# jianzhangcs/DAGL

Hardware: AMD Instinct MI355X
Metric: graph-attn fwd query-patches/s @256x256x64 k=8 (higher is better)
Workload: dtype f32

## Files before the change

### dagl_amd/csrc/prologue.hip

```cpp
#include <stdlib.h>

#include "dagl_common.h"
#include "thr_bias4.h"

namespace dagl {

constexpr int PC = 64;
constexpr int PRO_TW = 64;
constexpr int PRO_LW = PRO_TW + 2;
constexpr int PRO_LS = 68;
constexpr int PRO_ROWS = 4;

__global__ __launch_bounds__(256) void conv_pair_kernel(int H, int W, int rows_per_block,
                                                        const float* __restrict__ x,
                                                        const float* __restrict__ g_w, const float* __restrict__ g_b,
                                                        const float* __restrict__ th_w, const float* __restrict__ th_b,
                                                        float* __restrict__ b1p, float* __restrict__ b2p,
                                                        unsigned short* __restrict__ b1hi,
                                                        unsigned short* __restrict__ b1lo) {
    __shared__ __attribute__((aligned(16))) float ring[PRO_ROWS][PC][PRO_LS];
    const int tid = threadIdx.x;
    const int wave = __builtin_amdgcn_readfirstlane(tid >> 6);
    const int lane = tid & 63;
    const int i = lane & 15, g = lane >> 4;
    const int b = blockIdx.z;
    const int x0 = blockIdx.x * PRO_TW;
    const int y0 = blockIdx.y * rows_per_block;
    int y1 = y0 + rows_per_block; if (y1 > H) y1 = H;
    const int Hp = H + 2 * PADPIX, Wp = W + 2 * PADPIX;
    const float* xb = x + (size_t)b * PC * H * W;

    float wg[9][16], wt[16];
    {
        float* wl = &ring[0][0][0];
        for (int e = tid; e < 16 * PC * 9 / 4; e += 256)
            reinterpret_cast<float4*>(wl)[e] = reinterpret_cast<const float4*>(g_w)[e];
        for (int e = tid; e < 16 * PC / 4; e += 256)
            reinterpret_cast<float4*>(wl + 16 * PC * 9)[e] = reinterpret_cast<const float4*>(th_w)[e];
        __syncthreads();
#pragma unroll
        for (int tap = 0; tap < 9; ++tap)
#pragma unroll
            for (int T = 0; T < 16; ++T) wg[tap][T] = wl[(i * PC + 4 * T + g) * 9 + tap];
#pragma unroll
        for (int T = 0; T < 16; ++T) wt[T] = wl[16 * PC * 9 + i * PC + 4 * T + g];
        __syncthreads();
    }
    const float bias1 = g_b[i], bias2 = th_b[i];

    constexpr int NST = (PC * PRO_LW + 255) / 256;
    float st[NST];
    auto stage_load = [&](int yy) {
#pragma unroll
        for (int j = 0; j < NST; ++j) {
            const int idx = tid + 256 * j;
            const int ch = idx / PRO_LW, p = idx - ch * PRO_LW;
            const int xx = x0 - 1 + p;
            const bool ok = (idx < PC * PRO_LW) && (yy >= 0) && (yy < H) && (xx >= 0) && (xx < W);
            const int yc = yy < 0 ? 0 : (yy >= H ? H - 1 : yy), xc = xx < 0 ? 0 : (xx >= W ? W - 1 : xx);
            const int cc = ch < PC ? ch : PC - 1;
            const float raw = xb[((size_t)cc * H + yc) * W + xc];
            st[j] = ok ? raw : 0.f;
        }
    };
    auto stage_store = [&](int yy) {
        const int slot = (yy + 1) & (PRO_ROWS - 1);
#pragma unroll
        for (int j = 0; j < NST; ++j) {
            const int idx = tid + 256 * j;
            const int ch = idx / PRO_LW, p = idx - ch * PRO_LW;
            if (idx < PC * PRO_LW) ring[slot][ch][p] = st[j];
        }
    };

    stage_load(y0 - 1); stage_store(y0 - 1);
    stage_load(y0);     stage_store(y0);
    stage_load(y0 + 1); stage_store(y0 + 1);
    __syncthreads();

    const int px0 = 16 * wave;
    for (int y = y0; y < y1; ++y) {
        if (y + 1 < y1) stage_load(y + 2);
        f32x4 a0 = {0.f, 0.f, 0.f, 0.f}, a1 = a0, a2 = a0, at = a0;
#pragma unroll
        for (int T = 0; T < 16; ++T) {
            const int ch = 4 * T + g;
            const float* r0 = &ring[(y + 0) & 3][ch][px0 + i];
            const float* r1 = &ring[(y + 1) & 3][ch][px0 + i];
            const float* r2 = &ring[(y + 2) & 3][ch][px0 + i];
            const float c1 = r1[1];
            a0 = __builtin_amdgcn_mfma_f32_16x16x4f32(r0[0], wg[0][T], a0, 0, 0, 0);
            a1 = __builtin_amdgcn_mfma_f32_16x16x4f32(r1[0], wg[3][T], a1, 0, 0, 0);
            a2 = __builtin_amdgcn_mfma_f32_16x16x4f32(r2[0], wg[6][T], a2, 0, 0, 0);
            at = __builtin_amdgcn_mfma_f32_16x16x4f32(c1, wt[T], at, 0, 0, 0);
            a0 = __builtin_amdgcn_mfma_f32_16x16x4f32(r0[1], wg[1][T], a0, 0, 0, 0);
            a1 = __builtin_amdgcn_mfma_f32_16x16x4f32(c1, wg[4][T], a1, 0, 0, 0);
            a2 = __builtin_amdgcn_mfma_f32_16x16x4f32(r2[1], wg[7][T], a2, 0, 0, 0);
            a0 = __builtin_amdgcn_mfma_f32_16x16x4f32(r0[2], wg[2][T], a0, 0, 0, 0);
            a1 = __builtin_amdgcn_mfma_f32_16x16x4f32(r1[2], wg[5][T], a1, 0, 0, 0);
            a2 = __builtin_amdgcn_mfma_f32_16x16x4f32(r2[2], wg[8][T], a2, 0, 0, 0);
        }
#pragma unroll
        for (int r = 0; r < 4; ++r) {
            const int xx = x0 + px0 + 4 * g + r;
            if (xx < W) {
                const size_t o = (((size_t)b * Hp + y + PADPIX) * Wp + xx + PADPIX) * CH + i;
                const float v1 = ((a0[r] + a1[r]) + a2[r]) + bias1;
                if (b1p != nullptr) b1p[o] = v1;
                if (b1hi != nullptr) {
                    const float vs = v1 * 16.0f;
                    const _Float16 hh = (_Float16)vs;
                    const _Float16 ll = (_Float16)(vs - (float)hh);
                    b1hi[o] = __builtin_bit_cast(unsigned short, hh);
                    b1lo[o] = __builtin_bit_cast(unsigned short, ll);
                }
                b2p[o] = at[r] + bias2;
            }
        }
        if (y + 1 < y1) stage_store(y + 2);
        __syncthreads();
    }
}

typedef _Float16 h16x8 __attribute__((ext_vector_type(8)));
typedef _Float16 h16x4 __attribute__((ext_vector_type(4)));
constexpr int C16_PXB = 272;
constexpr int C16_ROWB = PRO_LW * C16_PXB;
constexpr int C16_WOFF = PRO_ROWS * C16_ROWB;
constexpr int C16_WB = (18 + 2) * 16 * 128;
constexpr float C16_XS = 16.0f, C16_WS = 256.0f;

__device__ __forceinline__ void c16_split(float v, _Float16& hi, _Float16& lo) {
    hi = (_Float16)v;
    lo = (_Float16)(v - (float)hi);
}

__global__ __launch_bounds__(256) void pack_conv_weight16_kernel(const float* __restrict__ g_w, const float* __restrict__ th_w,
                                                                 unsigned char* __restrict__ img) {
    const int e = blockIdx.x * 256 + threadIdx.x;
    if (e >= 16 * PC * 9 + 16 * PC) return;
    float v; int o, c, kb;
    if (e < 16 * PC * 9) {
        o = e / (PC * 9); const int rem = e - o * (PC * 9);
        c = rem / 9; const int tap = rem - c * 9;
        v = g_w[e]; kb = tap * 2 + (c >> 5);
    } else {
        const int t = e - 16 * PC * 9;
        o = t / PC; c = t - o * PC;
        v = th_w[t]; kb = 18 + (c >> 5);
    }
    _Float16 h, l;
    c16_split(v * C16_WS, h, l);
    unsigned char* d = img + (kb * 16 + o) * 128 + (c & 7) * 2;
    const int ks = (c & 31) >> 3, gs = (o >> 1) & 7;
    *reinterpret_cast<_Float16*>(d + ((ks ^ gs) << 4)) = h;
    *reinterpret_cast<_Float16*>(d + (((4 + ks) ^ gs) << 4)) = l;
    if (!(fabsf(v) * C16_WS < RANGE_LIMIT)) *reinterpret_cast<int32_t*>(img + C16_WB) = 1;
}

int launch_pack_conv_weight16(hipStream_t s, const float* g_w, const float* th_w, unsigned char* img) {
    DAGL_HIP_TRY(hipMemsetAsync(img + C16_WB, 0, 16, s));
    hipLaunchKernelGGL(pack_conv_weight16_kernel, dim3((16 * PC * 9 + 16 * PC + 255) / 256), dim3(256), 0, s, g_w, th_w, img);
    DAGL_LAUNCH_CHECK("pack_conv_weight16_kernel");
    return DAGL_OK;
}

__global__ __launch_bounds__(256) void conv_pair16_kernel(int H, int W, int rows_per_block, ConvHeadSet hs,
                                                          float* __restrict__ b2p, float* __restrict__ b1p, unsigned short* __restrict__ b1hi,
                                                          unsigned short* __restrict__ b1lo, uint32_t* __restrict__ clear_a,
                                                          int clear_a_words, uint32_t* __restrict__ clear_b, int clear_b_words,
                                                          RangeTag range, unsigned long long* times) {
    __shared__ __attribute__((aligned(16))) unsigned char smem[C16_WOFF + C16_WB + 16];
    int* const oor = reinterpret_cast<int*>(smem + C16_WOFF + C16_WB);
    const int tid = threadIdx.x;
    const int blin = (blockIdx.z * gridDim.y + blockIdx.y) * gridDim.x + blockIdx.x;
    dbg_stamp(times, blin, 0);
    float amax = 0.f;
    if (blockIdx.x == 0 && blockIdx.y == 0 && blockIdx.z == 0) {
        for (int t = tid; t < clear_a_words; t += 256) clear_a[t] = 0u;
        for (int t = tid; t < clear_b_words; t += 256) clear_b[t] = 0u;
    }
    if (tid == 0) *oor = 0;
    const int wave = __builtin_amdgcn_readfirstlane(tid >> 6);
    const int lane = tid & 63;
    const int i = lane & 15, kg = lane >> 4;
    const int b = blockIdx.z;
    const int head = b / hs.imgs;
    const float* __restrict__ x = hs.x[head];
    const unsigned char* __restrict__ wimg = hs.w[head];
    const float* __restrict__ g_b = hs.gb[head];
    const float* __restrict__ th_b = hs.tb[head];
    const int x0 = blockIdx.x * PRO_TW;
    const int y0 = blockIdx.y * rows_per_block;
    int y1 = y0 + rows_per_block; if (y1 > H) y1 = H;
    const int Hp = H + 2 * PADPIX, Wp = W + 2 * PADPIX;
    const float* xb = x + (size_t)(b - head * hs.imgs) * PC * H * W;

    const int hpx = 64 + (tid >> 6), hch = tid & 63;
    auto load_row = [&](int yy, float* st, float& sh) {
        const bool rok = (yy >= 0) && (yy < H);
        const int xa = x0 - 1 + lane, xc = x0 - 1 + hpx;
        const bool oka = rok && xa >= 0 && xa < W;
        const bool okc = rok && xc < W;
        const int yc = yy < 0 ? 0 : (yy >= H ? H - 1 : yy);
        const int xac = xa < 0 ? 0 : (xa >= W ? W - 1 : xa);
        const float* rp = xb + ((size_t)(16 * wave) * H + yc) * W + xac;
        float raw[16];
#pragma unroll
        for (int c = 0; c < 16; ++c) raw[c] = rp[(size_t)c * H * W];
        const float rh = xb[((size_t)hch * H + yc) * W + (xc >= W ? W - 1 : xc)];
#pragma unroll
        for (int c = 0; c < 16; ++c) st[c] = oka ? raw[c] : 0.f;
        sh = okc ? rh : 0.f;
    };
    float xs = C16_XS;
    float amax_x = 0.f;
    auto store_row = [&](int yy, const float* st, float sh) {
        unsigned char* row = smem + ((yy + 1) & (PRO_ROWS - 1)) * C16_ROWB;
        unsigned char* px = row + lane * C16_PXB;
        h16x8 hi0, hi1, lo0, lo1;
#pragma unroll
        for (int c = 0; c < 8; ++c) {
            _Float16 h, l;
            c16_split(st[c] * xs, h, l); hi0[c] = h; lo0[c] = l;
            c16_split(st[c + 8] * xs, h, l); hi1[c] = h; lo1[c] = l;
            amax_x = fmaxf(amax_x, fmaxf(fabsf(st[c]), fabsf(st[c + 8])));
        }
        *reinterpret_cast<h16x8*>(px + 32 * wave) = hi0;
        *reinterpret_cast<h16x8*>(px + 32 * wave + 16) = hi1;
        *reinterpret_cast<h16x8*>(px + 128 + 32 * wave) = lo0;
        *reinterpret_cast<h16x8*>(px + 128 + 32 * wave + 16) = lo1;
        if (tid < 128) {
            _Float16 h, l;
            c16_split(sh * xs, h, l);
            amax_x = fmaxf(amax_x, fabsf(sh));
            *reinterpret_cast<_Float16*>(row + hpx * C16_PXB + 2 * hch) = h;
            *reinterpret_cast<_Float16*>(row + hpx * C16_PXB + 128 + 2 * hch) = l;
        }
    };

    float st0[16], st1[16], st2[16], sh0, sh1, sh2;
    unsigned b1_bits = 0u;
    const bool tiers = hs.tiers.amax != nullptr;
    unsigned short* __restrict__ b1hi2 = hs.tiers.hi2;
    unsigned short* __restrict__ b1lo2 = hs.tiers.lo2;
    bool first = true;
    auto run_strip = [&]() {
    load_row(y0 - 1, st0, sh0);
    load_row(y0, st1, sh1);
    load_row(y0 + 1, st2, sh2);
    if (first) {
        uint4 wv[10];
#pragma unroll
        for (int j = 0; j < 10; ++j) wv[j] = reinterpret_cast<const uint4*>(wimg)[tid + 256 * j];
        if (tid == 0 && *reinterpret_cast<const int32_t*>(wimg + C16_WB) != 0) amax = __builtin_inff();
#pragma unroll
        for (int j = 0; j < 10; ++j) reinterpret_cast<uint4*>(smem + C16_WOFF)[tid + 256 * j] = wv[j];
    }
    store_row(y0 - 1, st0, sh0);
    store_row(y0, st1, sh1);
    store_row(y0 + 1, st2, sh2);
    __syncthreads();

    float bg[4], bt[4];
#pragma unroll
    for (int r = 0; r < 4; ++r) { bg[r] = g_b[4 * kg + r]; bt[r] = th_b[4 * kg + r]; }
    const unsigned char* wbase = smem + C16_WOFF + i * 128;
    const int whi = (kg ^ ((i >> 1) & 7)) << 4, wlo = ((4 + kg) ^ ((i >> 1) & 7)) << 4;
    const int pxo = (16 * wave + i) * C16_PXB + kg * 16;
    const float inv = 1.0f / (xs * C16_WS);
    h16x8 wh[20], wl2[20];
#pragma unroll
    for (int kb = 0; kb < 20; ++kb) {
        wh[kb] = *reinterpret_cast<const h16x8*>(wbase + kb * 2048 + whi);
        wl2[kb] = *reinterpret_cast<const h16x8*>(wbase + kb * 2048 + wlo);
    }
    b1_bits = 0u;

    dbg_stamp(times, blin, 1);
    if (y0 + 2 < y1 + 1) load_row(y0 + 2, st0, sh0);
    auto do_row = [&](int y, float* stc, float& shc, float* stn, float& shn) {
        if (y + 2 < y1) load_row(y + 3, stn, shn);
        f32x4 am[3][2], ac[3][2], tm[2], tc[2];
        const f32x4 zero4 = {0.f, 0.f, 0.f, 0.f};
#pragma unroll
        for (int u = 0; u < 3; ++u) { am[u][0] = zero4; am[u][1] = zero4; ac[u][0] = zero4; ac[u][1] = zero4; }
        tm[0] = zero4; tm[1] = zero4; tc[0] = zero4; tc[1] = zero4;
#pragma unroll
        for (int dx = 0; dx < 3; ++dx) {
#pragma unroll
            for (int dy = 0; dy < 3; ++dy) {
                const unsigned char* rowp = smem + ((y + dy) & (PRO_ROWS - 1)) * C16_ROWB + pxo;
#pragma unroll
                for (int cb = 0; cb < 2; ++cb) {
                    const int kb = (dy * 3 + dx) * 2 + cb;
                    const h16x8 w_hi = wh[kb], w_lo = wl2[kb];
                    const h16x8 p_hi = *reinterpret_cast<const h16x8*>(rowp + dx * C16_PXB + cb * 64);
                    const h16x8 p_lo = *reinterpret_cast<const h16x8*>(rowp + dx * C16_PXB + 128 + cb * 64);
                    ac[dy][cb] = __builtin_amdgcn_mfma_f32_16x16x32_f16(w_hi, p_lo, ac[dy][cb], 0, 0, 0);
                    am[dy][cb] = __builtin_amdgcn_mfma_f32_16x16x32_f16(w_hi, p_hi, am[dy][cb], 0, 0, 0);
                    ac[dy][cb] = __builtin_amdgcn_mfma_f32_16x16x32_f16(w_lo, p_hi, ac[dy][cb], 0, 0, 0);
                    if (dy == 1 && dx == 1) {
                        const h16x8 t_hi = wh[18 + cb], t_lo = wl2[18 + cb];
                        tc[cb] = __builtin_amdgcn_mfma_f32_16x16x32_f16(t_hi, p_lo, tc[cb], 0, 0, 0);
                        tm[cb] = __builtin_amdgcn_mfma_f32_16x16x32_f16(t_hi, p_hi, tm[cb], 0, 0, 0);
                        tc[cb] = __builtin_amdgcn_mfma_f32_16x16x32_f16(t_lo, p_hi, tc[cb], 0, 0, 0);
                    }
                }
            }
        }
        f32x4 ag, at;
#pragma unroll
        for (int r = 0; r < 4; ++r) {
            const float cr = ((ac[0][0][r] + ac[0][1][r]) + (ac[1][0][r] + ac[1][1][r])) + (ac[2][0][r] + ac[2][1][r]);
            const float mn = ((am[0][0][r] + am[0][1][r]) + (am[1][0][r] + am[1][1][r])) + (am[2][0][r] + am[2][1][r]);
            ag[r] = mn + cr;
            at[r] = (tm[0][r] + tm[1][r]) + (tc[0][r] + tc[1][r]);
        }
        const int xx = x0 + 16 * wave + i;
        if (xx < W) {
            const size_t o = (((size_t)b * Hp + y + PADPIX) * Wp + xx + PADPIX) * CH + 4 * kg;
            h16x4 vh, vl, vh2, vl2;
            float4 v2, v1q;
            float* v2p = &v2.x;
            float* v1p = &v1q.x;
#pragma unroll
            for (int r = 0; r < 4; ++r) {
                const float v1 = ag[r] * inv + bg[r];
                v1p[r] = v1;
                _Float16 h, l;
                c16_split(v1 * B1_FINE_SCALE, h, l);
                vh[r] = h; vl[r] = l;
                c16_split(v1 * B1_COARSE_SCALE, h, l);
                vh2[r] = h; vl2[r] = l;
                b1_bits = max(b1_bits, __float_as_uint(v1) & 0x7fffffffu);
                v2p[r] = at[r] * inv + bt[r];
            }
            if (b1hi != nullptr) {
                *reinterpret_cast<h16x4*>(b1hi + o) = vh;
                *reinterpret_cast<h16x4*>(b1lo + o) = vl;
            }
            if (b1p != nullptr) *reinterpret_cast<float4*>(b1p + o) = v1q;
            if (tiers && b1hi2 != nullptr) {
                *reinterpret_cast<h16x4*>(b1hi2 + o) = vh2;
                *reinterpret_cast<h16x4*>(b1lo2 + o) = vl2;
            }
            *reinterpret_cast<float4*>(b2p + o) = v2;
        }
        if (y + 1 < y1) store_row(y + 2, stc, shc);
        if (y + 1 >= y1 && !(amax_x * xs < RANGE_LIMIT)) *oor = 1;
        __syncthreads();
    };
    for (int y = y0; y < y1; y += 2) {
        do_row(y, st0, sh0, st1, sh1);
        if (y + 1 < y1) do_row(y + 1, st1, sh1, st0, sh0);
    }
    };
    run_strip();
    if (tiers && *oor != 0) {
        float m = amax_x;
#pragma unroll
        for (int o = 32; o > 0; o >>= 1) m = fmaxf(m, __shfl_xor(m, o));
        float* red = reinterpret_cast<float*>(smem);
        if (lane == 0) red[wave] = m;
        __syncthreads();
        m = fmaxf(fmaxf(red[0], red[1]), fmaxf(red[2], red[3]));
        __syncthreads();
        int e = 0;
        if (m <= 3.0e38f) { (void)frexpf(m, &e); e = 15 - e; }
        e = e < -120 ? -120 : (e > 4 ? 4 : e);
        xs = ldexpf(1.0f, e);
        first = false;
        run_strip();
    }
    dbg_stamp(times, blin, 2);
    if (tiers) {
        unsigned mb = b1_bits;
#pragma unroll
        for (int o = 32; o > 0; o >>= 1) mb = max(mb, (unsigned)__shfl_xor((int)mb, o));
        if (lane == 0) {
            const float m = mb >= 0x7f800000u ? __builtin_inff() : __uint_as_float(mb);
            const int img = b - head * hs.imgs;
            hs.tiers.amax[(size_t)head * hs.tiers.slots + (((size_t)img * gridDim.y + blockIdx.y) * gridDim.x + blockIdx.x) * 4 + wave] = m;
            if (range.word != nullptr && (!(m * B1_COARSE_SCALE < RANGE_LIMIT) || !(amax < RANGE_LIMIT))) *range.word = range.tag;
        }
    } else {
        if (range.word != nullptr && (!(amax < RANGE_LIMIT) || !(amax_x * xs < RANGE_LIMIT) || !((float)(b1_bits >= 0x7f800000u ? __builtin_inff() : __uint_as_float(b1_bits)) * B1_FINE_SCALE < RANGE_LIMIT)))
            *range.word = range.tag;
    }
    dbg_stamp(times, blin, 3);
}

int conv16_blocks_per_head(const Grid& g, int heads, int imgs) {
    const int B = heads * imgs;
    const int strips = (g.W + PRO_TW - 1) / PRO_TW;
    int chunks = (256 + strips * B - 1) / (strips * B);
    if (chunks > (g.H + 1) / 2) chunks = (g.H + 1) / 2;
    if (chunks < 1) chunks = 1;
    const int rows_per_block = (g.H + chunks - 1) / chunks;
    chunks = (g.H + rows_per_block - 1) / rows_per_block;
    return strips * chunks * imgs * 4;
}

constexpr int TB_XW = 4 * TB_Q + 4;
constexpr int TB_N = TB_CG * KS * TB_XW;
constexpr int TB_PER = (TB_N + 255) / 256;
__global__ __launch_bounds__(256) void thr_bias_kernel(Grid gr, ThrHeadSet hs,
                                                       float* __restrict__ part_out ) {
    __shared__ __attribute__((aligned(16))) float tile[TB_N + 256];
    __shared__ __attribute__((aligned(16))) float wl[2][TB_CG][KS][8];
    __shared__ float part[4][TB_Q][2];
    const int tid = threadIdx.x;
    const int lane = tid & 63, w = __builtin_amdgcn_readfirstlane(tid >> 6);
    const int qi = lane & 31, hh = lane >> 5;
    const int chunks = (gr.Lw + TB_Q - 1) / TB_Q;
    const int qr = blockIdx.x / chunks, q0 = (blockIdx.x - qr * chunks) * TB_Q;
    const int b = blockIdx.y, grp = blockIdx.z;
    const int head = b / hs.imgs, img = b - head * hs.imgs;
    const float* __restrict__ thr_w = hs.thr_w[head];
    const float* __restrict__ bias_w = hs.bias_w[head];
    const int c0 = grp * TB_CG;
    const int y0 = QS * qr - gr.pt, x0 = QS * q0 - gr.pl;
    const float* xc0 = hs.x[head] + ((size_t)img * PC + c0) * gr.N;
    float v[TB_PER];
#pragma unroll
    for (int j = 0; j < TB_PER; ++j) {
        const int idx = tid + 256 * j;
        const int c = idx / (KS * TB_XW), rem = idx - c * (KS * TB_XW);
        const int r = rem / TB_XW, col = rem - r * TB_XW;
        const int yy = y0 + r, xx = x0 + col;
        const int yc = yy < 0 ? 0 : (yy >= gr.H ? gr.H - 1 : yy), xc = xx < 0 ? 0 : (xx >= gr.W ? gr.W - 1 : xx);
        const int cc = c < TB_CG ? c : TB_CG - 1;
        v[j] = xc0[(size_t)cc * gr.N + yc * gr.W + xc];
    }
    for (int e = tid; e < TB_CG * KS * KS; e += 256) {
        const int ch = e / (KS * KS), t = e - ch * (KS * KS);
        const int kh = t / KS, kw = t - kh * KS;
        wl[0][ch][kh][kw] = thr_w[c0 * (KS * KS) + e];
        wl[1][ch][kh][kw] = bias_w[c0 * (KS * KS) + e];
    }
#pragma unroll
    for (int j = 0; j < TB_PER; ++j) {
        const int idx = tid + 256 * j;
        const int c = idx / (KS * TB_XW), rem = idx - c * (KS * TB_XW);
        const int r = rem / TB_XW, col = rem - r * TB_XW;
        const int yy = y0 + r, xx = x0 + col;
        const bool ok = yy >= 0 && yy < gr.H && xx >= 0 && xx < gr.W;
        tile[idx] = ok ? v[j] : 0.f;
    }
    __syncthreads();
    const int kh0 = hh ? 4 : 0, kh1 = hh ? KS : 4;
    float s1 = 0.f, s2 = 0.f;
#pragma unroll
    for (int j = 0; j < TB_CG / 4; ++j) {
        const int cl = 4 * j + w;
        for (int kh = kh0; kh < kh1; ++kh) {
            const float* rp = tile + (cl * KS + kh) * TB_XW + 4 * qi;
            const float4 v0 = *reinterpret_cast<const float4*>(rp);
            const float4 v1 = *reinterpret_cast<const float4*>(rp + 4);
            const float4 a0 = *reinterpret_cast<const float4*>(&wl[0][cl][kh][0]);
            const float4 a1 = *reinterpret_cast<const float4*>(&wl[0][cl][kh][4]);
            const float4 b0 = *reinterpret_cast<const float4*>(&wl[1][cl][kh][0]);
            const float4 b1 = *reinterpret_cast<const float4*>(&wl[1][cl][kh][4]);
            s1 = fmaf(v0.x, a0.x, s1); s1 = fmaf(v0.y, a0.y, s1); s1 = fmaf(v0.z, a0.z, s1); s1 = fmaf(v0.w, a0.w, s1);
            s1 = fmaf(v1.x, a1.x, s1); s1 = fmaf(v1.y, a1.y, s1); s1 = fmaf(v1.z, a1.z, s1);
            s2 = fmaf(v0.x, b0.x, s2); s2 = fmaf(v0.y, b0.y, s2); s2 = fmaf(v0.z, b0.z, s2); s2 = fmaf(v0.w, b0.w, s2);
            s2 = fmaf(v1.x, b1.x, s2); s2 = fmaf(v1.y, b1.y, s2); s2 = fmaf(v1.z, b1.z, s2);
        }
    }
    s1 += __shfl_xor(s1, 32); s2 += __shfl_xor(s2, 32);
    if (hh == 0) { part[w][qi][0] = s1; part[w][qi][1] = s2; }
    __syncthreads();
    if (tid < TB_Q && q0 + tid < gr.Lw) {
        const size_t o = (size_t)head * 8 * hs.imgs * gr.L + (((size_t)grp * hs.imgs + img) * gr.L + (size_t)qr * gr.Lw + q0 + tid) * 2;
        part_out[o] = (part[0][tid][0] + part[1][tid][0]) + (part[2][tid][0] + part[3][tid][0]);
        part_out[o + 1] = (part[0][tid][1] + part[1][tid][1]) + (part[2][tid][1] + part[3][tid][1]);
    }
}

__global__ __launch_bounds__(256) void thr_bias4_kernel(Grid gr, ThrHeadSet hs,
                                                        float* __restrict__ part_out ) {
    __shared__ __attribute__((aligned(16))) unsigned char smem[TB4_LDS_BYTES];
    thr_bias4_block(gr, hs, part_out, blockIdx.x, blockIdx.y, blockIdx.z, smem);
}

__global__ void thr_bias_reduce_kernel(size_t n , const float* __restrict__ part, const float* __restrict__ thr_b,
                                       const float* __restrict__ bias_b, float* __restrict__ thr, float* __restrict__ bias) {
    const size_t i = (size_t)blockIdx.x * blockDim.x + threadIdx.x;
    if (i >= n) return;
    const float2 p0 = reinterpret_cast<const float2*>(part)[i], p1 = reinterpret_cast<const float2*>(part)[n + i];
    const float2 p2 = reinterpret_cast<const float2*>(part)[2 * n + i], p3 = reinterpret_cast<const float2*>(part)[3 * n + i];
    thr[i] = ((p0.x + p1.x) + (p2.x + p3.x)) + thr_b[0];
    bias[i] = ((p0.y + p1.y) + (p2.y + p3.y)) + bias_b[0];
}

int launch_conv_pair16_heads(hipStream_t s, int heads, int imgs, const Grid& g, const ConvHeadSet& hs, float* b2p,
                             uint16_t* b1_hi, uint16_t* b1_lo, uint32_t* clear_a, int clear_a_words, uint32_t* clear_b,
                             int clear_b_words, RangeTag range) {
    const int B = heads * imgs;
    const int strips = (g.W + PRO_TW - 1) / PRO_TW;
    constexpr int target = 256;
    int chunks = (target + strips * B - 1) / (strips * B);
    if (chunks > (g.H + 1) / 2) chunks = (g.H + 1) / 2;
    if (chunks < 1) chunks = 1;
    const int rows_per_block = (g.H + chunks - 1) / chunks;
    chunks = (g.H + rows_per_block - 1) / rows_per_block;
    unsigned long long* times = nullptr;
#ifdef DAGL_ABLATION
    if (getenv("DAGL_TIMES_FILE")) times = dbg_times_buffer((size_t)strips * chunks * B);
#endif
    hipLaunchKernelGGL(conv_pair16_kernel, dim3(strips, chunks, B), dim3(256), 0, s, g.H, g.W, rows_per_block, hs,
                       b2p, (float*)nullptr, b1_hi, b1_lo, clear_a, clear_a_words, clear_b, clear_b_words, range, times);
    DAGL_LAUNCH_CHECK("conv_pair16_kernel");
#ifdef DAGL_ABLATION
    if (times) dbg_times_dump(s, "conv_pair16_kernel", times, (size_t)strips * chunks * B);
#endif
    return DAGL_OK;
}

int launch_thr_bias_heads(hipStream_t s, int heads, int imgs, const Grid& g, const ThrHeadSet& hs, float* thr_part) {
    const dim3 tb_grid(g.Lh * ((g.Lw + TB_Q - 1) / TB_Q), heads * imgs, TB_GROUPS);
    bool aligned = true;
    for (int h = 0; h < heads; ++h) aligned = aligned && (reinterpret_cast<uintptr_t>(hs.x[h]) & 15u) == 0;
    if (g.W % 4 == 0 && g.W >= 4 && g.pl == 1 && aligned)
        hipLaunchKernelGGL(thr_bias4_kernel, tb_grid, dim3(256), 0, s, g, hs, thr_part);
    else
        hipLaunchKernelGGL(thr_bias_kernel, tb_grid, dim3(256), 0, s, g, hs, thr_part);
    DAGL_LAUNCH_CHECK("thr_bias_kernel");
    return DAGL_OK;
}

int launch_prologue(hipStream_t s, int B, const Grid& g, const float* x, const float* g_w, const float* g_b,
                    const float* th_w, const float* th_b, const float* thr_w, const float* thr_b,
                    const float* bias_w, const float* bias_b, float* b1p, float* b2p, float* thr, float* bias,
                    uint16_t* b1_hi, uint16_t* b1_lo, float* thr_part, bool borders_zero, bool defer_thr_reduce, uint32_t* clear_a,
                    int clear_a_words, uint32_t* clear_b, int clear_b_words, RangeTag range, const unsigned char* conv_w16,
                    bool skip_conv, const B1Tiers* tiers) {
    int rcz;
    if (!borders_zero) {
        if ((rcz = launch_zero_borders(s, B, g.H, g.W, b1p ? b1p : b2p, b2p))) return rcz;
        if (b1_hi != nullptr && (rcz = launch_zero_borders16(s, B, g.H, g.W, b1_hi, b1_lo))) return rcz;
        if (b1_hi != nullptr && tiers != nullptr && tiers->hi2 != nullptr && (rcz = launch_zero_borders16(s, B, g.H, g.W, tiers->hi2, tiers->lo2))) return rcz;
    }
    const int strips = (g.W + PRO_TW - 1) / PRO_TW;
    constexpr int target = 256;
    int chunks = (target + strips * B - 1) / (strips * B);
    if (chunks > (g.H + 1) / 2) chunks = (g.H + 1) / 2;
    if (chunks < 1) chunks = 1;
    const int rows_per_block = (g.H + chunks - 1) / chunks;
    chunks = (g.H + rows_per_block - 1) / rows_per_block;
    if (skip_conv) {
    } else if ((b1p == nullptr && b1_hi != nullptr) || (b1p != nullptr && conv_w16 != nullptr)) {
        if (conv_w16 == nullptr) { set_error("launch_prologue: the split-fp16 convolutions need their packed weights"); return DAGL_ERR_INVALID; }
        ConvHeadSet hs = {};
        hs.x[0] = x; hs.w[0] = conv_w16; hs.gb[0] = g_b; hs.tb[0] = th_b; hs.imgs = B;
        if (tiers != nullptr) hs.tiers = *tiers;
        unsigned long long* times = nullptr;
#ifdef DAGL_ABLATION
        if (getenv("DAGL_TIMES_FILE")) times = dbg_times_buffer((size_t)strips * chunks * B);
#endif
        hipLaunchKernelGGL(conv_pair16_kernel, dim3(strips, chunks, B), dim3(256), 0, s, g.H, g.W, rows_per_block, hs,
                           b2p, b1p, b1_hi, b1_lo, clear_a, clear_a_words, clear_b, clear_b_words, range, times);
        DAGL_LAUNCH_CHECK("conv_pair16_kernel");
#ifdef DAGL_ABLATION
        if (times) dbg_times_dump(s, "conv_pair16_kernel", times, (size_t)strips * chunks * B);
#endif
    } else {
        hipLaunchKernelGGL(conv_pair_kernel, dim3(strips, chunks, B), dim3(256), 0, s, g.H, g.W, rows_per_block, x, g_w,
                           g_b, th_w, th_b, b1p, b2p, b1_hi, b1_lo);
        DAGL_LAUNCH_CHECK("conv_pair_kernel");
    }
    if (thr != nullptr) {
        if (!skip_conv) {
            ThrHeadSet hs = {};
            hs.x[0] = x; hs.thr_w[0] = thr_w; hs.bias_w[0] = bias_w; hs.imgs = B;
            const int rct = launch_thr_bias_heads(s, 1, B, g, hs, thr_part);
            if (rct) return rct;
        }
        const size_t n = (size_t)B * g.L;
        if (!defer_thr_reduce)
        hipLaunchKernelGGL(thr_bias_reduce_kernel, dim3((unsigned)((n + 255) / 256)), dim3(256), 0, s, n, thr_part, thr_b,
                           bias_b, thr, bias);
        DAGL_LAUNCH_CHECK("thr_bias_reduce_kernel");
    }
    return DAGL_OK;
}

}
```

Baseline: 18.23 million.

## Compute two output rows per pass in split-fp16 conv with deeper LDS ring

Restructures the split-fp16 MFMA convolution so each pass computes two output rows that share the four staged input rows, widening the LDS ring to six rows and prefetching two rows ahead. Weights are repacked into a lane-linear layout loaded straight into registers, and the weight global load is issued before the input-row loads. Input loads switch to buffer-resource loads with 32-bit offsets, and blocks are remapped in a strided order across the grid. The aim is to reuse each LDS pixel read for two rows, halve barriers per row and spread memory traffic, at the cost of more LDS, more accumulator registers and a new 4 GiB input-size limit.

New measurement: 18.32 million (median of 6 runs). About the same (+0.5%).

```diff
diff --git a/dagl_amd/csrc/prologue.hip b/dagl_amd/csrc/prologue.hip
--- a/dagl_amd/csrc/prologue.hip
+++ b/dagl_amd/csrc/prologue.hip
@@ -124,10 +124,11 @@
 
 typedef _Float16 h16x8 __attribute__((ext_vector_type(8)));
 typedef _Float16 h16x4 __attribute__((ext_vector_type(4)));
-constexpr int C16_PXB = 272;
+constexpr int C16_PXB = 288;
 constexpr int C16_ROWB = PRO_LW * C16_PXB;
-constexpr int C16_WOFF = PRO_ROWS * C16_ROWB;
-constexpr int C16_WB = (18 + 2) * 16 * 128;
+constexpr int C16_RING = 6;
+constexpr int C16_LDS = C16_RING * C16_ROWB;
+constexpr int C16_WB = (18 + 2) * 2 * 64 * 16;
 constexpr float C16_XS = 16.0f, C16_WS = 256.0f;
 
 __device__ __forceinline__ void c16_split(float v, _Float16& hi, _Float16& lo) {
@@ -151,10 +152,10 @@
     }
     _Float16 h, l;
     c16_split(v * C16_WS, h, l);
-    unsigned char* d = img + (kb * 16 + o) * 128 + (c & 7) * 2;
-    const int ks = (c & 31) >> 3, gs = (o >> 1) & 7;
-    *reinterpret_cast<_Float16*>(d + ((ks ^ gs) << 4)) = h;
-    *reinterpret_cast<_Float16*>(d + (((4 + ks) ^ gs) << 4)) = l;
+    const int lane = ((c & 31) >> 3) * 16 + o;
+    unsigned char* d = img + ((kb * 2) * 64 + lane) * 16 + (c & 7) * 2;
+    *reinterpret_cast<_Float16*>(d) = h;
+    *reinterpret_cast<_Float16*>(d + 64 * 16) = l;
     if (!(fabsf(v) * C16_WS < RANGE_LIMIT)) *reinterpret_cast<int32_t*>(img + C16_WB) = 1;
 }
 
@@ -170,8 +171,8 @@
                                                           unsigned short* __restrict__ b1lo, uint32_t* __restrict__ clear_a,
                                                           int clear_a_words, uint32_t* __restrict__ clear_b, int clear_b_words,
                                                           RangeTag range, unsigned long long* times) {
-    __shared__ __attribute__((aligned(16))) unsigned char smem[C16_WOFF + C16_WB + 16];
-    int* const oor = reinterpret_cast<int*>(smem + C16_WOFF + C16_WB);
+    __shared__ __attribute__((aligned(16))) unsigned char smem[C16_LDS + C16_WB + 16];
+    int* const oor = reinterpret_cast<int*>(smem + C16_LDS + C16_WB);
     const int tid = threadIdx.x;
     const int blin = (blockIdx.z * gridDim.y + blockIdx.y) * gridDim.x + blockIdx.x;
     dbg_stamp(times, blin, 0);
@@ -184,17 +185,28 @@
     const int wave = __builtin_amdgcn_readfirstlane(tid >> 6);
     const int lane = tid & 63;
     const int i = lane & 15, kg = lane >> 4;
-    const int b = blockIdx.z;
+    int tx = blockIdx.x, ty = blockIdx.y, tb = blockIdx.z;
+    {
+        const int nb = gridDim.x * gridDim.y * gridDim.z;
+        if ((nb & 7) == 0) {
+            const int lin = (blockIdx.z * gridDim.y + blockIdx.y) * gridDim.x + blockIdx.x;
+            const int t = (lin & 7) * (nb >> 3) + (lin >> 3);
+            tx = t % gridDim.x; ty = (t / gridDim.x) % gridDim.y; tb = t / (gridDim.x * gridDim.y);
+        }
+    }
+    const int b = tb;
     const int head = b / hs.imgs;
     const float* __restrict__ x = hs.x[head];
     const unsigned char* __restrict__ wimg = hs.w[head];
     const float* __restrict__ g_b = hs.gb[head];
     const float* __restrict__ th_b = hs.tb[head];
-    const int x0 = blockIdx.x * PRO_TW;
-    const int y0 = blockIdx.y * rows_per_block;
+    const int x0 = tx * PRO_TW;
+    const int y0 = ty * rows_per_block;
     int y1 = y0 + rows_per_block; if (y1 > H) y1 = H;
     const int Hp = H + 2 * PADPIX, Wp = W + 2 * PADPIX;
     const float* xb = x + (size_t)(b - head * hs.imgs) * PC * H * W;
+    const unsigned HW4 = (unsigned)H * W * 4;
+    const __amdgpu_buffer_rsrc_t xrs = __builtin_amdgcn_make_buffer_rsrc(const_cast<float*>(xb), (short)0, (int)(PC * HW4), 0x00020000);
 
     const int hpx = 64 + (tid >> 6), hch = tid & 63;
     auto load_row = [&](int yy, float* st, float& sh) {
@@ -204,19 +216,22 @@
         const bool okc = rok && xc < W;
         const int yc = yy < 0 ? 0 : (yy >= H ? H - 1 : yy);
         const int xac = xa < 0 ? 0 : (xa >= W ? W - 1 : xa);
-        const float* rp = xb + ((size_t)(16 * wave) * H + yc) * W + xac;
+        const unsigned vo = ((unsigned)yc * W + xac) * 4;
         float raw[16];
 #pragma unroll
-        for (int c = 0; c < 16; ++c) raw[c] = rp[(size_t)c * H * W];
-        const float rh = xb[((size_t)hch * H + yc) * W + (xc >= W ? W - 1 : xc)];
+        for (int c = 0; c < 16; ++c)
+            raw[c] = __builtin_bit_cast(float, __builtin_amdgcn_raw_buffer_load_b32(xrs, (int)vo, (int)((16 * wave + c) * HW4), 0));
+        const float rh = __builtin_bit_cast(float, __builtin_amdgcn_raw_buffer_load_b32(
+                             xrs, (int)(((unsigned)hch * H * W + (unsigned)yc * W + (xc >= W ? W - 1 : xc)) * 4), 0, 0));
 #pragma unroll
         for (int c = 0; c < 16; ++c) st[c] = oka ? raw[c] : 0.f;
         sh = okc ? rh : 0.f;
     };
     float xs = C16_XS;
     float amax_x = 0.f;
+    auto slot = [&](int yy) { return ((yy + 1) % C16_RING) * C16_ROWB; };
     auto store_row = [&](int yy, const float* st, float sh) {
-        unsigned char* row = smem + ((yy + 1) & (PRO_ROWS - 1)) * C16_ROWB;
+        unsigned char* row = smem + slot(yy);
         unsigned char* px = row + lane * C16_PXB;
         h16x8 hi0, hi1, lo0, lo1;
 #pragma unroll
@@ -239,83 +254,78 @@
         }
     };
 
-    float st0[16], st1[16], st2[16], sh0, sh1, sh2;
+    float st0[16], st1[16], st2[16], st3[16], sh0, sh1, sh2, sh3;
     unsigned b1_bits = 0u;
     const bool tiers = hs.tiers.amax != nullptr;
     unsigned short* __restrict__ b1hi2 = hs.tiers.hi2;
     unsigned short* __restrict__ b1lo2 = hs.tiers.lo2;
     bool first = true;
     auto run_strip = [&]() {
+    uint4 wv[10];
+    if (first) {
+#pragma unroll
+        for (int j = 0; j < 10; ++j) wv[j] = reinterpret_cast<const uint4*>(wimg)[tid + 256 * j];
+    }
     load_row(y0 - 1, st0, sh0);
     load_row(y0, st1, sh1);
     load_row(y0 + 1, st2, sh2);
+    if (y0 + 1 < y1) load_row(y0 + 2, st3, sh3);
+    h16x8 wh[20], wl2[20];
     if (first) {
-        uint4 wv[10];
-#pragma unroll
-        for (int j = 0; j < 10; ++j) wv[j] = reinterpret_cast<const uint4*>(wimg)[tid + 256 * j];
         if (tid == 0 && *reinterpret_cast<const int32_t*>(wimg + C16_WB) != 0) amax = __builtin_inff();
 #pragma unroll
-        for (int j = 0; j < 10; ++j) reinterpret_cast<uint4*>(smem + C16_WOFF)[tid + 256 * j] = wv[j];
+        for (int j = 0; j < 10; ++j) reinterpret_cast<uint4*>(smem + C16_LDS)[tid + 256 * j] = wv[j];
     }
     store_row(y0 - 1, st0, sh0);
     store_row(y0, st1, sh1);
     store_row(y0 + 1, st2, sh2);
+    if (y0 + 1 < y1) store_row(y0 + 2, st3, sh3);
     __syncthreads();
+    {
+        const h16x8* wsrc = reinterpret_cast<const h16x8*>(smem + C16_LDS) + lane;
+#pragma unroll
+        for (int kb = 0; kb < 20; ++kb) {
+            wh[kb] = wsrc[(2 * kb) * 64];
+            wl2[kb] = wsrc[(2 * kb + 1) * 64];
+        }
+    }
 
     float bg[4], bt[4];
 #pragma unroll
     for (int r = 0; r < 4; ++r) { bg[r] = g_b[4 * kg + r]; bt[r] = th_b[4 * kg + r]; }
-    const unsigned char* wbase = smem + C16_WOFF + i * 128;
-    const int whi = (kg ^ ((i >> 1) & 7)) << 4, wlo = ((4 + kg) ^ ((i >> 1) & 7)) << 4;
     const int pxo = (16 * wave + i) * C16_PXB + kg * 16;
     const float inv = 1.0f / (xs * C16_WS);
-    h16x8 wh[20], wl2[20];
-#pragma unroll
-    for (int kb = 0; kb < 20; ++kb) {
-        wh[kb] = *reinterpret_cast<const h16x8*>(wbase + kb * 2048 + whi);
-        wl2[kb] = *reinterpret_cast<const h16x8*>(wbase + kb * 2048 + wlo);
-    }
     b1_bits = 0u;
 
     dbg_stamp(times, blin, 1);
-    if (y0 + 2 < y1 + 1) load_row(y0 + 2, st0, sh0);
-    auto do_row = [&](int y, float* stc, float& shc, float* stn, float& shn) {
-        if (y + 2 < y1) load_row(y + 3, stn, shn);
-        f32x4 am[3][2], ac[3][2], tm[2], tc[2];
+    struct Acc { f32x4 am[3][2], ac[3][2], tm[2], tc[2]; };
+    auto zero = [&](Acc& a) {
         const f32x4 zero4 = {0.f, 0.f, 0.f, 0.f};
 #pragma unroll
-        for (int u = 0; u < 3; ++u) { am[u][0] = zero4; am[u][1] = zero4; ac[u][0] = zero4; ac[u][1] = zero4; }
-        tm[0] = zero4; tm[1] = zero4; tc[0] = zero4; tc[1] = zero4;
-#pragma unroll
-        for (int dx = 0; dx < 3; ++dx) {
-#pragma unroll
-            for (int dy = 0; dy < 3; ++dy) {
-                const unsigned char* rowp = smem + ((y + dy) & (PRO_ROWS - 1)) * C16_ROWB + pxo;
-#pragma unroll
-                for (int cb = 0; cb < 2; ++cb) {
-                    const int kb = (dy * 3 + dx) * 2 + cb;
-                    const h16x8 w_hi = wh[kb], w_lo = wl2[kb];
-                    const h16x8 p_hi = *reinterpret_cast<const h16x8*>(rowp + dx * C16_PXB + cb * 64);
-                    const h16x8 p_lo = *reinterpret_cast<const h16x8*>(rowp + dx * C16_PXB + 128 + cb * 64);
-                    ac[dy][cb] = __builtin_amdgcn_mfma_f32_16x16x32_f16(w_hi, p_lo, ac[dy][cb], 0, 0, 0);
-                    am[dy][cb] = __builtin_amdgcn_mfma_f32_16x16x32_f16(w_hi, p_hi, am[dy][cb], 0, 0, 0);
-                    ac[dy][cb] = __builtin_amdgcn_mfma_f32_16x16x32_f16(w_lo, p_hi, ac[dy][cb], 0, 0, 0);
-                    if (dy == 1 && dx == 1) {
-                        const h16x8 t_hi = wh[18 + cb], t_lo = wl2[18 + cb];
-                        tc[cb] = __builtin_amdgcn_mfma_f32_16x16x32_f16(t_hi, p_lo, tc[cb], 0, 0, 0);
-                        tm[cb] = __builtin_amdgcn_mfma_f32_16x16x32_f16(t_hi, p_hi, tm[cb], 0, 0, 0);
-                        tc[cb] = __builtin_amdgcn_mfma_f32_16x16x32_f16(t_lo, p_hi, tc[cb], 0, 0, 0);
-                    }
-                }
-            }
-        }
+        for (int u = 0; u < 3; ++u) { a.am[u][0] = zero4; a.am[u][1] = zero4; a.ac[u][0] = zero4; a.ac[u][1] = zero4; }
+        a.tm[0] = zero4; a.tm[1] = zero4; a.tc[0] = zero4; a.tc[1] = zero4;
+    };
+    auto mul = [&](Acc& a, int dy, int dx, int cb, const h16x8& p_hi, const h16x8& p_lo) {
+        const int kb = (dy * 3 + dx) * 2 + cb;
+        const h16x8 w_hi = wh[kb], w_lo = wl2[kb];
+        a.ac[dy][cb] = __builtin_amdgcn_mfma_f32_16x16x32_f16(w_hi, p_lo, a.ac[dy][cb], 0, 0, 0);
+        a.am[dy][cb] = __builtin_amdgcn_mfma_f32_16x16x32_f16(w_hi, p_hi, a.am[dy][cb], 0, 0, 0);
+        a.ac[dy][cb] = __builtin_amdgcn_mfma_f32_16x16x32_f16(w_lo, p_hi, a.ac[dy][cb], 0, 0, 0);
+        if (dy == 1 && dx == 1) {
+            const h16x8 t_hi = wh[18 + cb], t_lo = wl2[18 + cb];
+            a.tc[cb] = __builtin_amdgcn_mfma_f32_16x16x32_f16(t_hi, p_lo, a.tc[cb], 0, 0, 0);
+            a.tm[cb] = __builtin_amdgcn_mfma_f32_16x16x32_f16(t_hi, p_hi, a.tm[cb], 0, 0, 0);
+            a.tc[cb] = __builtin_amdgcn_mfma_f32_16x16x32_f16(t_lo, p_hi, a.tc[cb], 0, 0, 0);
+        }
+    };
+    auto emit = [&](int y, const Acc& a) {
         f32x4 ag, at;
 #pragma unroll
         for (int r = 0; r < 4; ++r) {
-            const float cr = ((ac[0][0][r] + ac[0][1][r]) + (ac[1][0][r] + ac[1][1][r])) + (ac[2][0][r] + ac[2][1][r]);
-            const float mn = ((am[0][0][r] + am[0][1][r]) + (am[1][0][r] + am[1][1][r])) + (am[2][0][r] + am[2][1][r]);
+            const float cr = ((a.ac[0][0][r] + a.ac[0][1][r]) + (a.ac[1][0][r] + a.ac[1][1][r])) + (a.ac[2][0][r] + a.ac[2][1][r]);
+            const float mn = ((a.am[0][0][r] + a.am[0][1][r]) + (a.am[1][0][r] + a.am[1][1][r])) + (a.am[2][0][r] + a.am[2][1][r]);
             ag[r] = mn + cr;
-            at[r] = (tm[0][r] + tm[1][r]) + (tc[0][r] + tc[1][r]);
+            at[r] = (a.tm[0][r] + a.tm[1][r]) + (a.tc[0][r] + a.tc[1][r]);
         }
         const int xx = x0 + 16 * wave + i;
         if (xx < W) {
@@ -347,14 +357,58 @@
             }
             *reinterpret_cast<float4*>(b2p + o) = v2;
         }
-        if (y + 1 < y1) store_row(y + 2, stc, shc);
-        if (y + 1 >= y1 && !(amax_x * xs < RANGE_LIMIT)) *oor = 1;
+    };
+    auto do_pair = [&](int y) {
+        const bool more = y + 2 < y1;
+        const bool more2 = y + 3 < y1;
+        if (more) load_row(y + 3, st0, sh0);
+        if (more2) load_row(y + 4, st1, sh1);
+        Acc a0, a1;
+        zero(a0); zero(a1);
+#pragma unroll
+        for (int dx = 0; dx < 3; ++dx) {
+#pragma unroll
+            for (int r = 0; r < 4; ++r) {
+                const unsigned char* rowp = smem + slot(y - 1 + r) + pxo;
+#pragma unroll
+                for (int cb = 0; cb < 2; ++cb) {
+                    const h16x8 p_hi = *reinterpret_cast<const h16x8*>(rowp + dx * C16_PXB + cb * 64);
+                    const h16x8 p_lo = *reinterpret_cast<const h16x8*>(rowp + dx * C16_PXB + 128 + cb * 64);
+                    if (r < 3) mul(a0, r, dx, cb, p_hi, p_lo);
+                    if (r > 0) mul(a1, r - 1, dx, cb, p_hi, p_lo);
+                }
+            }
+        }
+        emit(y, a0);
+        emit(y + 1, a1);
+        if (more) store_row(y + 3, st0, sh0);
+        if (more2) store_row(y + 4, st1, sh1);
+        if (!more && !(amax_x * xs < RANGE_LIMIT)) *oor = 1;
         __syncthreads();
     };
-    for (int y = y0; y < y1; y += 2) {
-        do_row(y, st0, sh0, st1, sh1);
-        if (y + 1 < y1) do_row(y + 1, st1, sh1, st0, sh0);
-    }
+    auto do_row = [&](int y) {
+        Acc a;
+        zero(a);
+#pragma unroll
+        for (int dx = 0; dx < 3; ++dx) {
+#pragma unroll
+            for (int dy = 0; dy < 3; ++dy) {
+                const unsigned char* rowp = smem + slot(y - 1 + dy) + pxo;
+#pragma unroll
+                for (int cb = 0; cb < 2; ++cb) {
+                    const h16x8 p_hi = *reinterpret_cast<const h16x8*>(rowp + dx * C16_PXB + cb * 64);
+                    const h16x8 p_lo = *reinterpret_cast<const h16x8*>(rowp + dx * C16_PXB + 128 + cb * 64);
+                    mul(a, dy, dx, cb, p_hi, p_lo);
+                }
+            }
+        }
+        emit(y, a);
+        if (!(amax_x * xs < RANGE_LIMIT)) *oor = 1;
+        __syncthreads();
+    };
+    int yr = y0;
+    for (; yr + 1 < y1; yr += 2) do_pair(yr);
+    if (yr < y1) do_row(yr);
     };
     run_strip();
     if (tiers && *oor != 0) {
@@ -381,7 +435,7 @@
         if (lane == 0) {
             const float m = mb >= 0x7f800000u ? __builtin_inff() : __uint_as_float(mb);
             const int img = b - head * hs.imgs;
-            hs.tiers.amax[(size_t)head * hs.tiers.slots + (((size_t)img * gridDim.y + blockIdx.y) * gridDim.x + blockIdx.x) * 4 + wave] = m;
+            hs.tiers.amax[(size_t)head * hs.tiers.slots + (((size_t)img * gridDim.y + ty) * gridDim.x + tx) * 4 + wave] = m;
             if (range.word != nullptr && (!(m * B1_COARSE_SCALE < RANGE_LIMIT) || !(amax < RANGE_LIMIT))) *range.word = range.tag;
         }
     } else {
@@ -494,9 +548,16 @@
     bias[i] = ((p0.y + p1.y) + (p2.y + p3.y)) + bias_b[0];
 }
 
+static bool conv16_fits(const Grid& g) {
+    if ((size_t)PC * g.H * g.W * 4 < ((size_t)1 << 32)) return true;
+    set_error("conv_pair16_kernel: an image's input must stay below 4 GiB");
+    return false;
+}
+
 int launch_conv_pair16_heads(hipStream_t s, int heads, int imgs, const Grid& g, const ConvHeadSet& hs, float* b2p,
                              uint16_t* b1_hi, uint16_t* b1_lo, uint32_t* clear_a, int clear_a_words, uint32_t* clear_b,
                              int clear_b_words, RangeTag range) {
+    if (!conv16_fits(g)) return DAGL_ERR_INVALID;
     const int B = heads * imgs;
     const int strips = (g.W + PRO_TW - 1) / PRO_TW;
     constexpr int target = 256;
@@ -552,6 +613,7 @@
     if (skip_conv) {
     } else if ((b1p == nullptr && b1_hi != nullptr) || (b1p != nullptr && conv_w16 != nullptr)) {
         if (conv_w16 == nullptr) { set_error("launch_prologue: the split-fp16 convolutions need their packed weights"); return DAGL_ERR_INVALID; }
+        if (!conv16_fits(g)) return DAGL_ERR_INVALID;
         ConvHeadSet hs = {};
         hs.x[0] = x; hs.w[0] = conv_w16; hs.gb[0] = g_b; hs.tb[0] = th_b; hs.imgs = B;
         if (tiers != nullptr) hs.tiers = *tiers;
```
